# cwchenwang/outdoor-nerf-depth

Measured on AMD Instinct MI355X. Metric: train rays/sec, KITTI 375x1242, 64+128 samples/ray, higher is better.
Workload: dtype bf16 MFMA operands, f32 accumulate / f32 master weights

## Files before the change

### outdoor_nerf_depth_amd/csrc/nerfpp_common.h

```cpp
#pragma once
#include <stdint.h>
#ifdef NERFPP_PROBES
#include <stdlib.h>
#endif

namespace nerfpp {

constexpr int WIDTH = 256;
constexpr int FRAG_BYTES = 1024;
constexpr int BLK_FRAGS = 16;
constexpr int DIR_REF = 27;
constexpr int DIRW = 32;
constexpr int N_NET = 2;

__host__ __device__ constexpr int pe_dim(int net) { return net == 0 ? 3 : 4; }
__host__ __device__ constexpr int pe_ref_ch(int net) { return net == 0 ? 63 : 84; }
__host__ __device__ constexpr int kpe(int net) { return net == 0 ? 4 : 6; }
__host__ __device__ constexpr int kpew(int net) { return kpe(net) * 16; }

enum RefTensor { RT_L0 = 0, RT_SIGMA = 8, RT_REMAP = 9, RT_RGB0 = 10, RT_RGB1 = 11, RT_COUNT = 12 };
__host__ __device__ constexpr int ref_out(int t) {
  return t < 8 ? 256 : t == RT_SIGMA ? 1 : t == RT_REMAP ? 256 : t == RT_RGB0 ? 128 : 3;
}
__host__ __device__ constexpr int ref_in(int net, int t) {
  return t == 0 ? pe_ref_ch(net) : t == 5 ? pe_ref_ch(net) + 256 : t < 8 ? 256
       : t == RT_SIGMA ? 256 : t == RT_REMAP ? 256 : t == RT_RGB0 ? 256 + DIR_REF : 128;
}
__host__ __device__ constexpr int ref_w_off(int net, int t) {
  int off = 0;
  for (int i = 0; i < t; ++i) off += ref_out(i) * ref_in(net, i) + ref_out(i);
  return off;
}
__host__ __device__ constexpr int ref_b_off(int net, int t) {
  return ref_w_off(net, t) + ref_out(t) * ref_in(net, t);
}
__host__ __device__ constexpr int net_params(int net) { return ref_w_off(net, RT_COUNT); }
constexpr int FG_PARAMS = net_params(0);
constexpr int BG_PARAMS = net_params(1);
constexpr int LEVEL_PARAMS = FG_PARAMS + BG_PARAMS;
static_assert(FG_PARAMS == 595844 && BG_PARAMS == 606596, "reference parameter count");

enum FwdStage { FS_L0 = 0, FS_L5 = 5, FS_REMAP = 8, FS_SIG = 9, FS_RGB0 = 10, FS_RGB1 = 11, FS_COUNT = 12 };
__host__ __device__ constexpr int fs_nob(int s) { return s <= FS_REMAP ? 8 : s == FS_RGB0 ? 4 : 1; }
__host__ __device__ constexpr int fs_nkc(int net, int s) {
  return s == FS_L0 ? kpe(net) : s == FS_L5 ? kpe(net) + 16 : s == FS_REMAP ? 0 : s < FS_REMAP ? 16
       : s == FS_SIG ? 16 : s == FS_RGB0 ? 20 : 16;
}
constexpr int DERIVED_WC = 128 * 256;
constexpr int DERIVED_FLOATS = DERIVED_WC + 128;
__host__ __device__ constexpr int fs_frags(int net, int s) { return fs_nob(s) * fs_nkc(net, s); }
__host__ __device__ constexpr int fs_frag_off(int net, int s) {
  int off = 0;
  for (int i = 0; i < s; ++i) off += fs_frags(net, i);
  return off;
}
__host__ __device__ constexpr int fs_bias_off(int s) {
  int off = 0;
  for (int i = 0; i < s; ++i) off += fs_nob(i) * 32;
  return off;
}
__host__ __device__ constexpr int fwd_frags(int net) { return fs_frag_off(net, FS_COUNT); }
constexpr int FWD_BIAS_FLOATS = fs_bias_off(FS_COUNT);
static_assert(fwd_frags(0) % BLK_FRAGS == 0 && fwd_frags(1) % BLK_FRAGS == 0, "block aligned");

enum BwdStage { BS_DG = 0, BS_DR = 1, BS_DH7 = 2, BS_COUNT = 10 };
__host__ __device__ constexpr int bs_nob(int s) { return s == BS_DG ? 4 : 8; }
__host__ __device__ constexpr int bs_nkc(int s) { return s == BS_DG ? 4 : s == BS_DR ? 0 : s == BS_DH7 ? 10 : 16; }
__host__ __device__ constexpr int bs_frags(int s) { return bs_nob(s) * bs_nkc(s); }
__host__ __device__ constexpr int bs_frag_off(int s) {
  int off = 0;
  for (int i = 0; i < s; ++i) off += bs_frags(i);
  return off;
}
constexpr int BWD_FRAGS = bs_frag_off(BS_COUNT);
static_assert(BWD_FRAGS % BLK_FRAGS == 0, "block aligned");
__host__ __device__ constexpr int bs_layer(int s) { return 10 - s; }

__host__ __device__ constexpr int w_planes(int P) { return P == 1 ? 1 : 2; }
__host__ __device__ constexpr int a_planes(int P) { return P == 2 ? 2 : 1; }
__host__ __device__ constexpr size_t fwd_stream_bytes(int net, int P) { return (size_t)fwd_frags(net) * FRAG_BYTES * w_planes(P); }
__host__ __device__ constexpr size_t bwd_stream_bytes(int P) { return (size_t)BWD_FRAGS * FRAG_BYTES * w_planes(P); }

__host__ __device__ constexpr int kslot(int c, int hi, int t) { return 16 * c + 8 * (t >> 2) + 4 * hi + (t & 3); }
__host__ __device__ constexpr int dfeat(int ob, int hi, int r) { return ob * 32 + (r & 3) + 8 * (r >> 2) + 4 * hi; }

__host__ __device__ constexpr int pe_ref_of_lane_slot(int D, int hi, int m) {
  const int nf = 10 * D;
  if (m < nf) {
    const int k = 5 * hi + m / (2 * D), d = (m % (2 * D)) / 2, s = m & 1;
    return D + k * 2 * D + s * D + d;
  }
  const int id = 2 * hi + (m - nf);
  return (m - nf) < 2 && id < D ? id : -1;
}
__host__ __device__ constexpr int dir_ref_of_lane_slot(int hi, int m) {
  if (m < 12) {
    const int k = 2 * hi + m / 6, d = (m % 6) / 2, s = m & 1;
    return 3 + k * 6 + s * 3 + d;
  }
  const int id = 2 * hi + (m - 12);
  return (m - 12) < 2 && id < 3 ? id : -1;
}
__host__ __device__ constexpr int feat_hi(int f) { return ((f % 16) / 4) % 2; }
__host__ __device__ constexpr int feat_m(int f) { return 8 * (f / 16) + 4 * ((f % 16) / 8) + (f % 4); }
__host__ __device__ constexpr int pe_ref_of_feat(int net, int f) { return pe_ref_of_lane_slot(pe_dim(net), feat_hi(f), feat_m(f)); }
__host__ __device__ constexpr int dir_ref_of_feat(int f) { return dir_ref_of_lane_slot(feat_hi(f), feat_m(f)); }

enum Tensor {
  T_X = 0, T_H0 = 1,  T_R = 9, T_G = 10, T_DIRX = 11,
  T_DZ0 = 12,  T_DR = 20, T_DS = 21, T_DG = 22, T_DP = 23, T_COUNT = 24
};
constexpr int DSG_LD = 160, DG_COL0 = 32;
__host__ __device__ constexpr int tensor_ld(int net, int t) {
  return t == T_X ? kpew(net) : (t >= T_H0 && t <= T_R) ? 256 : t == T_G ? 128 : t == T_DIRX ? 32
       : (t >= T_DZ0 && t <= T_DR) ? 256 : (t == T_DS || t == T_DG) ? DSG_LD : 32;
}
__host__ __device__ constexpr int tensor_off_cols(int net, int t) {
  int off = 0;
  for (int i = 0; i < t; ++i) off += tensor_ld(net, i);
  return off;
}
__host__ __device__ constexpr int ws_cols(int net) { return tensor_off_cols(net, T_COUNT); }

__host__ __device__ constexpr int gw_O(int s) { return s <= FS_REMAP ? 256 : s == FS_SIG ? 32 : s == FS_RGB0 ? 128 : 32; }
__host__ __device__ constexpr int gw_I(int net, int s) {
  return s == FS_L0 ? kpew(net) : s == FS_L5 ? kpew(net) + 256 : s <= FS_SIG ? 256 : s == FS_RGB0 ? 256 + DIRW : 128;
}
__host__ __device__ constexpr int gw_off(int net, int s) {
  int off = 0;
  for (int i = 0; i < s; ++i) off += gw_O(i) * gw_I(net, i);
  return off;
}
__host__ __device__ constexpr int gw_floats(int net) { return gw_off(net, FS_COUNT); }
__host__ __device__ constexpr int gb_off(int s) {
  int off = 0;
  for (int i = 0; i < s; ++i) off += gw_O(i);
  return off;
}
constexpr int GB_FLOATS = gb_off(FS_COUNT);
__host__ __device__ constexpr int gslab_floats(int net) { return gw_floats(net) + GB_FLOATS; }
__host__ __device__ constexpr int gw_dz_tensor(int s) {
  return s < 8 ? T_DZ0 + s : s == FS_REMAP ? T_DR : s == FS_SIG ? T_DS : s == FS_RGB0 ? T_DG : T_DP;
}

struct DwJob {
  int16_t a_tensor, b_tensor;
  int16_t b_tensor2, n_i1;
  int16_t o0, i0;
  int16_t n_o, n_i;
  int32_t gw_off;
  int16_t gw_ld;
  int16_t gb_off;
  int16_t o_split;
  int16_t gw_ld2, gb_off2;
  int32_t gw_off2;
};
constexpr int DW_JOBS = 10;
constexpr int DW_KMAX = 64;

// ... 161 lines not shown
```

### outdoor_nerf_depth_amd/csrc/nerfpp_mlp.hip

```cpp
#include <hip/hip_runtime.h>
#include <math.h>
#include <stdint.h>
#include <type_traits>
#include <utility>
#include "hip_device.h"
#include "nerfpp_common.h"
#include "nerfpp_kernels.h"

#ifdef NERFPP_PROBES
#include "nerfpp_mlp_probes.h"
#else
namespace nerfpp { namespace probe {
constexpr int STAMP_BYTES = 0;
__device__ __forceinline__ void stamp(int, int, int, int, uint32_t) {}
__device__ __forceinline__ void dump_stamps(uint32_t, int, int) {}
}}
#endif

namespace nerfpp {

using hipdev::bf16x8, hipdev::bf16x2, hipdev::f16x8, hipdev::f16x2, hipdev::f32x2, hipdev::f32x4, hipdev::f32x8, hipdev::f32x16;
using hipdev::u32x4, hipdev::s16x2, hipdev::s16x8, hipdev::glds16xN_saddr;
#define LDS_AS __attribute__((address_space(3)))

template <int P> struct Frag { bf16x8 v[a_planes(P)]; };

extern __shared__ __attribute__((aligned(16))) char smem[];

enum { PIPE_RING = 1, PIPE_ROLES = 2 };

__device__ __forceinline__ uint32_t lds_base_addr() { return (uint32_t)(uintptr_t)(LDS_AS char*)smem; }

template <int P, int NW, int MODE, int NBUF, int BF = BLK_FRAGS>
struct WeightPipe {
  static constexpr int BLKF = BF;
  static constexpr int BLK_BYTES = BF * P * FRAG_BYTES;
  static constexpr int SHARE = MODE == PIPE_ROLES ? BF * P : BF * P / NW;
  static constexpr int AHEAD = NBUF - 1;
  static_assert(AHEAD >= 1 && AHEAD <= 3 && (AHEAD - 1) * SHARE < 63, "ring depth");
  const char* g;
  uint32_t stamp_off = 0;
  int nblk, cur, step, wave, lane;
  int slot_cur, slot_issue, next_issue;
  uint32_t lds_base;
  __device__ __forceinline__ void init(const void* stream, int nblk_, int wave_, int lane_) {
    g = (const char*)stream; nblk = nblk_; cur = 0; step = 0; wave = wave_; lane = lane_;
    slot_cur = 0; slot_issue = 0; next_issue = 0;
    lds_base = lds_base_addr();
#pragma unroll
    for (int b = 0; b < AHEAD; ++b) issue();
  }
  static constexpr bool TRICKLE = MODE == PIPE_RING && AHEAD >= 2;
  int pend_blk = -1, pend_slot = 0;
  __device__ __forceinline__ void issue_frags(int blk, int slot, int f0, int f1) {
    if (MODE == PIPE_ROLES && wave != 0) return;
    const int w0 = MODE == PIPE_ROLES ? 0 : wave * SHARE;
    const char* sb = g + (size_t)blk * BLK_BYTES + (size_t)w0 * FRAG_BYTES;
    const uint32_t dst = lds_base + slot * BLK_BYTES + w0 * FRAG_BYTES;
#pragma unroll
    for (int f = f0; f < f1; f += 4) {
      const int n = f1 - f < 4 ? f1 - f : 4;
      const char* a = sb + f * FRAG_BYTES;
      const uint32_t d = dst + f * FRAG_BYTES;
      if (n == 4) glds16xN_saddr<4>(a, (uint32_t)lane * 16u, d);
      else if (n == 3) glds16xN_saddr<3>(a, (uint32_t)lane * 16u, d);
      else if (n == 2) glds16xN_saddr<2>(a, (uint32_t)lane * 16u, d);
      else glds16xN_saddr<1>(a, (uint32_t)lane * 16u, d);
    }
  }
  __device__ __forceinline__ bool claim(int& blk, int& slot) {
    blk = next_issue; slot = slot_issue;
    ++next_issue;
    slot_issue = slot_issue + 1 == NBUF ? 0 : slot_issue + 1;
    return blk < nblk;
  }
  __device__ __forceinline__ void issue() {
    int blk, slot;
    if (!claim(blk, slot)) return;
    static_assert(SHARE == 2 || SHARE % 4 == 0, "per-wave fragment count");
    issue_frags(blk, slot, 0, SHARE);
  }
  __device__ __forceinline__ void trickle(int i, int n) {
    if constexpr (TRICKLE) {
      if (pend_blk < 0) return;
      issue_frags(pend_blk, pend_slot, SHARE * i / n, SHARE * (i + 1) / n);
    }
  }
  __device__ __forceinline__ void wait_counted() {
    const int younger = nblk - 1 - step < AHEAD - 1 ? nblk - 1 - step : AHEAD - 1;
    if (AHEAD >= 3 && younger >= 2) asm volatile("s_waitcnt vmcnt(%0)" ::"n"(2 * SHARE) : "memory");
    else if (AHEAD >= 2 && younger == 1) asm volatile("s_waitcnt vmcnt(%0)" ::"n"(SHARE) : "memory");
    else asm volatile("s_waitcnt vmcnt(0)" ::: "memory");
  }
  __device__ __forceinline__ void sync_step() {
    probe::stamp(0, cur, wave, lane, stamp_off);
    if constexpr (MODE == PIPE_RING) {
      wait_counted();
      __builtin_amdgcn_s_barrier();
    } else {
      if (wave == 0) wait_counted();
      asm volatile("s_waitcnt lgkmcnt(0)" ::: "memory");
      __builtin_amdgcn_s_barrier();
    }
    probe::stamp(1, cur, wave, lane, stamp_off);
    if constexpr (TRICKLE) { int b_, s_; pend_blk = claim(b_, s_) ? b_ : -1; pend_slot = s_; }
    else issue();
    ++step;
  }
  __device__ __forceinline__ const char* acquire() {
    sync_step();
    const char* l = smem + slot_cur * BLK_BYTES + lane * 16;
    slot_cur = slot_cur + 1 == NBUF ? 0 : slot_cur + 1;
    ++cur;
    return l;
  }
};

template <int P>
__device__ __forceinline__ void mfma_p(f32x16& acc, const char* lfrag, const Frag<P>& b) {
  const bf16x8 a_hi = *(const bf16x8*)(lfrag);
  if constexpr (P == 3) {
    const bf16x8 a_lo = *(const bf16x8*)(lfrag + FRAG_BYTES);
    const f16x8 bb = __builtin_bit_cast(f16x8, b.v[0]);
    acc = __builtin_amdgcn_mfma_f32_32x32x16_f16(__builtin_bit_cast(f16x8, a_hi), bb, acc, 0, 0, 0);
    acc = __builtin_amdgcn_mfma_f32_32x32x16_f16(__builtin_bit_cast(f16x8, a_lo), bb, acc, 0, 0, 0);
  } else {
    acc = __builtin_amdgcn_mfma_f32_32x32x16_bf16(a_hi, b.v[0], acc, 0, 0, 0);
  }
}

struct NoHook { __device__ __forceinline__ void operator()(int) const {} };
#define HOOK(...) [&](int blk) __attribute__((always_inline)) { __VA_ARGS__; }
#define IC(n) std::integral_constant<int, (n)>{}

constexpr int LDS_PREFETCH = 4;
constexpr int LDS_PREFETCH_SPLIT = 4;
constexpr int CHAIN_GROUP = 4;

template <int NOB, int NKC, int P, int LIVE = NKC, typename Pipe, typename Hook>
__device__ __forceinline__ void stage_gemm(Pipe& pipe, f32x16 (&acc)[NOB], const Frag<P> (&b)[NKC], const Hook& hook) {
  static_assert(P == 1 || P == 3, "split-bf16 runs stage_units (nerfpp_mlp_split.h)");
  constexpr int KPB = Pipe::BLKF / NOB;
  static_assert(NKC % KPB == 0, "stage must be block aligned");
  static_assert(LIVE >= 1 && LIVE <= NKC, "live k-chunks");
#pragma unroll
// ... 118 lines not shown
      }
      const s16x8 zero = {0, 0, 0, 0, 0, 0, 0, 0};
      h[2 * ob + hh].v[0] = __builtin_bit_cast(bf16x8, __builtin_elementwise_max(__builtin_bit_cast(s16x8, d), zero));
    }
  return make_uint4(m[0], m[1], m[2], m[3]);
}

template <int N, int P>
__device__ __forceinline__ void zero_invalid(Frag<P> (&f)[N], bool valid) {
#pragma unroll
  for (int c = 0; c < N; ++c)
#pragma unroll
    for (int p = 0; p < a_planes(P); ++p) {
      u32x4 d = __builtin_bit_cast(u32x4, f[c].v[p]);
#pragma unroll
      for (int w = 0; w < 4; ++w) d[w] = valid ? d[w] : 0u;
      f[c].v[p] = __builtin_bit_cast(bf16x8, d);
    }
}

template <int NOB>
__device__ __forceinline__ void init_bias_lds(f32x16 (&acc)[NOB], uint32_t lds_off_bytes, int hi) {
  LDS_AS char* base = (LDS_AS char*)smem;
#pragma unroll
  for (int ob = 0; ob < NOB; ++ob) {
#pragma unroll
    for (int q = 0; q < 4; ++q) {
      const f32x4 v = *(LDS_AS f32x4*)(base + lds_off_bytes + (ob * 32 + hi * 16 + 4 * q) * 4);
      acc[ob][4 * q] = v[0]; acc[ob][4 * q + 1] = v[1]; acc[ob][4 * q + 2] = v[2]; acc[ob][4 * q + 3] = v[3];
    }
  }
}
template <int NOB>
__device__ __forceinline__ void init_zero(f32x16 (&acc)[NOB]) {
#pragma unroll
  for (int ob = 0; ob < NOB; ++ob)
#pragma unroll
    for (int r = 0; r < 16; ++r) acc[ob][r] = 0.f;
}

__device__ __forceinline__ void store_nt16(char* gptr, const uint4 v) {
  const u32x4 vv = {v.x, v.y, v.z, v.w};
  __builtin_nontemporal_store(vv, (u32x4*)gptr);
}

constexpr int REGION_MASK = 16 * FRAG_BYTES;
constexpr int REGION_BYTES = REGION_MASK + 1024;

__device__ __forceinline__ char* frag_addr(__bf16* base, int ld, size_t wave_row0, int c, int lane) {
  const size_t blk = (wave_row0 >> 5) * (size_t)(ld >> 4) + (size_t)c;
  return (char*)base + blk * FRAG_BYTES + ((((lane & 31) << 1) | (lane >> 5)) << 4);
}
template <int P>
__device__ __forceinline__ void store_chunk(__bf16* base, size_t plane, int ld, size_t wave_row0, int lane, int c, const Frag<P>& f, int np = a_planes(P)) {
#pragma unroll
  for (int p = 0; p < a_planes(P); ++p)
    if (p < np) store_nt16(frag_addr(base + p * plane, ld, wave_row0, c, lane), saved_image<P>(*(const uint4*)&f.v[p]));
}
template <int NCH, int P>
__device__ __forceinline__ void save_frags(__bf16* base, size_t plane, int ld, size_t wave_row0, int lane, const Frag<P> (&h)[NCH], int np = a_planes(P)) {
  __builtin_amdgcn_sched_barrier(0);
#pragma unroll
  for (int c = 0; c < NCH; ++c) store_chunk<P>(base, plane, ld, wave_row0, lane, c, h[c], np);
  __builtin_amdgcn_sched_barrier(0);
}

template <int NCH, int P>
__device__ __forceinline__ void handoff_write(char* region, int lane, const Frag<P> (&h)[NCH]) {
  static_assert(a_planes(P) == 1, "one plane");
#pragma unroll
  for (int c = 0; c < NCH; ++c) *(uint4*)(region + (c * 64 + lane) * 16) = *(const uint4*)&h[c].v[0];
}
template <int P>
__device__ __forceinline__ void handoff_flush_one(const char* region, int lane, __bf16* base, int ld, size_t row0, int cr, int ct) {
  static_assert(a_planes(P) == 1, "one plane");
  store_nt16(frag_addr(base, ld, row0, ct, lane), saved_image<P>(*(const uint4*)(region + (cr * 64 + lane) * 16)));
}
template <int P>
__device__ __forceinline__ void handoff_flush_chunks(const char* region, int lane, __bf16* base, int ld, size_t row0, int c0, int n) {
#pragma unroll 4
  for (int c = c0; c < c0 + n; ++c) handoff_flush_one<P>(region, lane, base, ld, row0, c, c);
}

template <int NOB>
__device__ __forceinline__ void mask_to_frags(const f32x16 (&acc)[NOB], const uint4 bits, Frag<1> (&dz)[2 * NOB]) {
  const uint32_t act[4] = {~bits.x, ~bits.y, ~bits.z, ~bits.w};
#pragma unroll
  for (int ob = 0; ob < NOB; ++ob)
#pragma unroll
    for (int hh = 0; hh < 2; ++hh) {
      u32x4 d;
#pragma unroll
      for (int w = 0; w < 4; ++w) d[w] = pack2<1>(acc[ob][8 * hh + 2 * w], acc[ob][8 * hh + 2 * w + 1]);
#pragma unroll
      for (int w = 0; w < 4; ++w) {
        const int j = (ob & 1) * 8 + hh * 4 + w;
        const s16x2 keep = __builtin_bit_cast(s16x2, act[ob >> 1] << j) >> (s16x2){15, 15};
        d[w] &= __builtin_bit_cast(uint32_t, keep);
      }
      dz[2 * ob + hh].v[0] = __builtin_bit_cast(bf16x8, d);
    }
}

template <int NET>
__device__ __forceinline__ void sample_point(const MlpGeom& gm, size_t row, int S, float (&x)[4], float (&vd)[3],
                                             float* depth_real) {
#pragma clang fp contract(off)
  const int ray = (int)(row / S);
  const float ox = gm.ray_o[ray * 3], oy = gm.ray_o[ray * 3 + 1], oz = gm.ray_o[ray * 3 + 2];
  const float dx = gm.ray_d[ray * 3], dy = gm.ray_d[ray * 3 + 1], dz = gm.ray_d[ray * 3 + 2];
  const float z = gm.z[row];
  const float dd = dx * dx + dy * dy + dz * dz;
  const float inv_n = 1.f / sqrtf(dd);
  vd[0] = dx * inv_n; vd[1] = dy * inv_n; vd[2] = dz * inv_n;
  if (NET == 0) {
    x[0] = ox + z * dx; x[1] = oy + z * dy; x[2] = oz + z * dz; x[3] = 0.f;
    *depth_real = 0.f;
  } else {
    const float d1 = -(dx * ox + dy * oy + dz * oz) / dd;
    const float mx = ox + d1 * dx, my = oy + d1 * dy, mz = oz + d1 * dz;
    const float pmn = sqrtf(mx * mx + my * my + mz * mz);
    const float d2 = sqrtf(1.f - pmn * pmn) * inv_n;
    const float sx = ox + (d1 + d2) * dx, sy = oy + (d1 + d2) * dy, sz = oz + (d1 + d2) * dz;
    float ax = oy * sz - oz * sy, ay = oz * sx - ox * sz, az = ox * sy - oy * sx;
    const float an = 1.f / sqrtf(ax * ax + ay * ay + az * az);
    ax *= an; ay *= an; az *= an;
    const float phi = asinf(pmn), theta = asinf(pmn * z);
    float sn, cs;
    sincosf(phi - theta, &sn, &cs);
    const float cx = ay * sz - az * sy, cy = az * sx - ax * sz, cz = ax * sy - ay * sx;
    const float dt = (ax * sx + ay * sy + az * sz) * (1.f - cs);
    float nx = sx * cs + cx * sn + ax * dt, ny = sy * cs + cy * sn + ay * dt, nz = sz * cs + cz * sn + az * dt;
    const float nn = 1.f / sqrtf(nx * nx + ny * ny + nz * nz);
    x[0] = nx * nn; x[1] = ny * nn; x[2] = nz * nn; x[3] = z;
    *depth_real = 1.f / (z + 1e-6f) * cosf(theta) * inv_n + d1;
  }
}

template <int P>
__device__ __forceinline__ void pe_sincos(float arg, float* sn, float* cs) {
#pragma clang fp contract(off)
  if constexpr (P != 2) {
    const float r = __builtin_amdgcn_fractf(arg * 0.15915494309189535f);
    *sn = __builtin_amdgcn_sinf(r);
    *cs = __builtin_amdgcn_cosf(r);
  } else {
    const float n = __builtin_rintf(arg * 0.6366197723675814f);
    float r = __builtin_fmaf(-n, 1.5707962512969971f, arg);
    r = __builtin_fmaf(-n, 7.5497901264043321e-08f, r);
    r = __builtin_fmaf(-n, -1.7763568394002505e-15f, r);
    const float z = r * r;
    float ps = __builtin_fmaf(z, 2.7183114e-6f, -0.00019839335f);
    ps = __builtin_fmaf(z, ps, 0.008333329f);
    ps = __builtin_fmaf(z, ps, -0.16666667f);
    const float s = __builtin_fmaf(r * z, ps, r);
    float pc = __builtin_fmaf(z, 2.4390449e-5f, -0.0013886763f);
    pc = __builtin_fmaf(z, pc, 0.04166662f);
    pc = __builtin_fmaf(z, pc, -0.5f);
    const float c = __builtin_fmaf(z, pc, 1.0f);
    const int q = (int)n;
    const float ss = (q & 1) ? c : s, cc = (q & 1) ? s : c;
    *sn = (q & 2) ? -ss : ss;
    *cs = ((q + 1) & 2) ? -cc : cc;
  }
}

template <int NET, int P>
__device__ __forceinline__ void encode_point(const float (&x)[4], int hi, Frag<P> (&pe)[kpe(NET)]) {
#pragma clang fp contract(off)
  constexpr int D = pe_dim(NET), NV = kpe(NET) * 8;
  float v[NV];
#pragma unroll
  for (int kk = 0; kk < 5; ++kk) {
    const float scale = __int_as_float((127 + 5 * hi + kk) << 23);
#pragma unroll
    for (int d = 0; d < D; ++d) {
      float sn, cs;
      pe_sincos<P>(x[d] * scale, &sn, &cs);
      v[(kk * D + d) * 2] = sn;
      v[(kk * D + d) * 2 + 1] = cs;
    }
  }
  v[10 * D] = hi ? x[2] : x[0];
  v[10 * D + 1] = hi ? (D == 4 ? x[3] : 0.f) : x[1];
// ... 200 lines not shown
      for (int c = 0; c < KPE; ++c) in5[c] = pe2[c];
    }
#pragma unroll
    for (int c = 0; c < 16; ++c) in5[KPE + c] = h[c];
    bias_init8(acc, fs_bias_off(FS_L5));
    stage_gemm<8, KPE + 16, P>(pipe, acc, in5, HOOK(psave_h(blk, h, a.ws.t[T_H0 + 4], 4)));
    const uint4 bits = acc_to_frags_relu_bits<8, P>(acc, h);
    finish_h(h, bits, 5);
  }
  for (int l = 6; l <= 7; ++l) {
    bias_init8(acc, fs_bias_off(FS_L0) + l * 256);
    stage_gemm<8, 16, P>(pipe, acc, h, HOOK(psave_h(blk, h, a.ws.t[T_H0 + l - 1], l - 1)));
    const uint4 bits = acc_to_frags_relu_bits<8, P>(acc, h);
    finish_h(h, bits, l);
  }
  f32x16 acc1[1];
  bias_init1(acc1, fs_bias_off(FS_SIG));
  constexpr int SIG_BLKS = P == 1 ? 1 : 0;
  stage_gemm<1, 16, P>(pipe, acc1, h, HOOK(if constexpr (P == 1) psave_hc(blk, h, a.ws.t[T_H0 + 7], 7, IC(3))));
  const float sigma_raw = acc1[0][0];
  Frag<P> g[8];
  {
    Frag<P> in[20];
#pragma unroll
    for (int c = 0; c < 16; ++c) in[c] = h[c];
    Frag<P> df[2];
    encode_dir<P>(vd, hi, df);
    in[16] = df[0]; in[17] = df[1]; in[18] = zero_frag<P>(); in[19] = zero_frag<P>();
    f32x16 acc4[4];
    bias_init4(acc4, fs_bias_off(FS_RGB0));
    stage_gemm<4, 20, P, 18>(pipe, acc4, in, HOOK(psave_hc(blk + SIG_BLKS, h, a.ws.t[T_H0 + 7], 7, IC(P == 1 ? 3 : 2))));
    const uint4 bits = acc_to_frags_relu_bits<4, P>(acc4, g);
    save(std::integral_constant<int, 8>{}, a.ws.t[T_G], 128, g, true, bits, 8);
  }
  {
    Frag<P> in[16];
#pragma unroll
    for (int c = 0; c < 8; ++c) in[c] = g[c];
#pragma unroll
    for (int c = 8; c < 16; ++c) in[c] = zero_frag<P>();
    bias_init1(acc1, fs_bias_off(FS_RGB1));
    stage_gemm<1, 16, P, 8>(pipe, acc1, in, HOOK(flush(blk, IC(8), a.ws.t[T_G], 128, 8)));
  }
  if (valid && hi == 0) {
    float4 o;
    o.x = 1.f / (1.f + expf(-acc1[0][0]));
    o.y = 1.f / (1.f + expf(-acc1[0][1]));
    o.z = 1.f / (1.f + expf(-acc1[0][2]));
    o.w = sigma_raw;
    ((float4*)a.out_raw)[row] = o;
    if (NET == 1) a.depth_real[row] = depth_real;
  }
  probe::dump_stamps(LD::TOTAL, wave, lane);
}

template <int NET, int NW>
__device__ __forceinline__ void mlp_bwd_body(const MlpBwdArgs& a, const int bid) {
  constexpr int P = 1;
  using LD = BwdLds<NW>;
  const int lane = threadIdx.x & 63, wave = __builtin_amdgcn_readfirstlane(threadIdx.x >> 6);
  const int hi = lane >> 5;
  const size_t row_raw = (size_t)bid * (NW * 32) + wave * 32 + (lane & 31);
  const bool valid = row_raw < (size_t)a.rows;
  const size_t row = valid ? row_raw : (size_t)a.rows - 1;
  const size_t plane_rows = a.rows_padded;
  const size_t wrow0 = (size_t)bid * (NW * 32) + wave * 32;
  const bool loader = wave == 0, partner = wave == 1;
  char* region = smem + LD::REGION;
  const size_t tile_row0 = wrow0 - (size_t)wave * 32;
  const size_t nblk32 = a.rows_padded / 32;
  const uint32_t lds0 = lds_base_addr();

  auto issue_masks = [&](int mstage) __attribute__((always_inline)) {
    if (loader && mstage >= 0) {
      static_assert(NW % 4 == 0, "groups of four");
      const char* sb = (const char*)(a.masks + ((size_t)mstage * nblk32 + (size_t)bid * NW) * 64);
#pragma unroll
      for (int w = 0; w < NW; w += 4) glds16xN_saddr<4>(sb + w * 1024, (uint32_t)lane * 16u, lds0 + LD::MASKS + ((mstage & 1) * NW + w) * 1024);
    }
  };
  auto get_mask = [&](int mstage) __attribute__((always_inline)) -> uint4 {
    return *(const uint4*)(smem + LD::MASKS + ((mstage & 1) * NW + wave) * 1024 + lane * 16);
  };
  auto psave = [&](int blk, auto nch_c, const auto& frags, __bf16* base, int ld) __attribute__((always_inline)) {
    constexpr int NCH = decltype(nch_c)::value, HMAX = NW >= 5 ? 4 : NW - 1, HN = NCH / 4 < HMAX ? NCH / 4 : HMAX;
    constexpr int Q = (NCH + HN - 1) / HN, CPB = LD::BF / 8;
    if (a.skip_dz7 && base == a.ws.t[T_DZ0 + 7]) return;
    if (loader) {
      if (blk == 0) handoff_write<NCH, P>(region, lane, frags);
    } else {
      if (CPB * blk < NCH) {
#pragma unroll
        for (int i = 0; i < CPB; ++i)
          store_chunk<P>(base, plane_rows * ld, ld, wrow0, lane, CPB * blk + i, frags[CPB * blk + i]);
      }
      if (wave <= HN && blk == 2) handoff_flush_chunks<P>(region, lane, base, ld, tile_row0, Q * (wave - 1), Q);
    }
  };

  issue_masks(8);
  issue_masks(7);
  WeightPipe<P, NW, PIPE_ROLES, LD::NBUF, LD::BF> pipe;
  pipe.stamp_off = LD::TOTAL;
  pipe.init(a.w_stream, BWD_FRAGS / LD::BF, wave, lane);

  float4 d = ((const float4*)a.d_out)[row];
  if (!valid) d = make_float4(0.f, 0.f, 0.f, 0.f);
  auto save_dp_ds = [&](const float4& dd, size_t r0) __attribute__((always_inline)) {
    Frag<P> t[2];
    t[0] = zero_frag<P>(); t[1] = zero_frag<P>();
    if (hi == 0) { set_slot<P>(t[0], 0, dd.x); set_slot<P>(t[0], 1, dd.y); set_slot<P>(t[0], 2, dd.z); }
    save_frags<2, P>(a.ws.t[T_DP], plane_rows * 32, 32, r0, lane, t);
    t[0] = zero_frag<P>();
    if (hi == 0) set_slot<P>(t[0], 0, dd.w);
    save_frags<2, P>(a.ws.t[T_DS], plane_rows * DSG_LD, DSG_LD, r0, lane, t);
  };
  {
    const size_t rr = row_raw - 32;
    const bool ok = partner && rr < (size_t)a.rows;
    float4 d0 = make_float4(0.f, 0.f, 0.f, 0.f);
    if (ok) d0 = ((const float4*)a.d_out)[rr];
    if (!loader) save_dp_ds(d, wrow0);
    if (partner) save_dp_ds(d0, wrow0 - 32);
  }

  Frag<P> dg[8];
  {
    Frag<P> in[4];
#pragma unroll
    for (int c = 0; c < 4; ++c) in[c] = zero_frag<P>();
    if (hi == 0) { set_slot<P>(in[0], 0, d.x); set_slot<P>(in[0], 1, d.y); set_slot<P>(in[0], 2, d.z); }
    f32x16 acc4[4];
    init_zero<4>(acc4);
    stage_gemm<4, 4, P, 1>(pipe, acc4, in, NoHook{});
    mask_to_frags<4>(acc4, get_mask(8), dg);
  }
  f32x16 acc[8];
  Frag<P> dz[16];
  {
    Frag<P> in[10];
#pragma unroll
    for (int c = 0; c < 8; ++c) in[c] = dg[c];
    in[8] = zero_frag<P>(); in[9] = zero_frag<P>();
    if (hi == 0) set_slot<P>(in[8], 0, d.w);
    init_zero<8>(acc);
    stage_gemm<8, 10, P, 9>(pipe, acc, in, HOOK(psave(blk, IC(8), dg, a.ws.t[T_DG], DSG_LD); if (blk == 0) issue_masks(6)));
    mask_to_frags<8>(acc, get_mask(7), dz);
  }
  for (int l = 7; l >= 1; --l) {
    init_zero<8>(acc);
    stage_gemm<8, 16, P>(pipe, acc, dz, HOOK(psave(blk, IC(16), dz, a.ws.t[T_DZ0 + l], 256); if (blk == 0) issue_masks(l - 2)));
    mask_to_frags<8>(acc, get_mask(l - 1), dz);
  }
  save_frags<16, P>(a.ws.t[T_DZ0], plane_rows * 256, 256, wrow0, lane, dz);
  probe::dump_stamps(LD::TOTAL, wave, lane);
}

}
#include "nerfpp_mlp_split.h"
namespace nerfpp {

template <int P, int NW, bool TRAIN>
__global__ __launch_bounds__(NW * 64, (NW == 8 ? 2 : 1)) void mlp_fwd_pair_kernel(MlpFwdArgs a0, MlpFwdArgs a1, int tiles0) {
  if constexpr (P == 2) {
    const bool fg = (int)blockIdx.x < tiles0;
    const bool hi_only = TRAIN && !(fg ? a0.save_lo : a1.save_lo);
    if (fg) { if (hi_only) mlp_fwd_body_split<0, NW, TRAIN, TRAIN>(a0, (int)blockIdx.x); else mlp_fwd_body_split<0, NW, TRAIN, false>(a0, (int)blockIdx.x); }
    else { if (hi_only) mlp_fwd_body_split<1, NW, TRAIN, TRAIN>(a1, (int)blockIdx.x - tiles0); else mlp_fwd_body_split<1, NW, TRAIN, false>(a1, (int)blockIdx.x - tiles0); }
  } else {
    if ((int)blockIdx.x < tiles0) mlp_fwd_body<0, P, NW, TRAIN>(a0, (int)blockIdx.x);
    else mlp_fwd_body<1, P, NW, TRAIN>(a1, (int)blockIdx.x - tiles0);
  }
}
template <int P, int NW>
__global__ __launch_bounds__(NW * 64, (P == 1 ? 2 : 1)) void mlp_bwd_pair_kernel(MlpBwdArgs a0, MlpBwdArgs a1, int tiles0) {
  if constexpr (P == 2) {
    if ((int)blockIdx.x < tiles0) mlp_bwd_body_split<0, NW>(a0, (int)blockIdx.x);
    else mlp_bwd_body_split<1, NW>(a1, (int)blockIdx.x - tiles0);
  } else {
    if ((int)blockIdx.x < tiles0) mlp_bwd_body<0, NW>(a0, (int)blockIdx.x);
    else mlp_bwd_body<1, NW>(a1, (int)blockIdx.x - tiles0);
  }
}

}

using namespace nerfpp;

constexpr int WAVES_P1 = 8;
#define MLP_WAVES(P) ((P) == 1 ? WAVES_P1 : (P) == 3 ? 8 : 4)

template <int P, bool TRAIN>
static void launch_fwd_t(hipStream_t st, const MlpFwdArgs& a0, const MlpFwdArgs& a1, int which) {
  constexpr int NW = MLP_WAVES(P);
  const int tile = NW * 32;
  const int t0 = which == 2 ? 0 : (int)((a0.rows + tile - 1) / tile), t1 = which == 1 ? 0 : (int)((a1.rows + tile - 1) / tile);
  constexpr size_t l0 = FwdLds<0, P, NW, TRAIN>::TOTAL, l1 = FwdLds<1, P, NW, TRAIN>::TOTAL;
  constexpr size_t lds = (l0 > l1 ? l0 : l1) + probe::STAMP_BYTES;
  static_assert(lds <= 160 * 1024, "LDS budget");
  hipLaunchKernelGGL((mlp_fwd_pair_kernel<P, NW, TRAIN>), dim3(t0 + t1), dim3(NW * 64), lds, st, a0, a1, t0);
}
template <int P>
static void launch_bwd_t(hipStream_t st, const MlpBwdArgs& a0, const MlpBwdArgs& a1, int which) {
  constexpr int NW = MLP_WAVES(P);
  const int tile = NW * 32;
  const int t0 = which == 2 ? 0 : (int)((a0.rows + tile - 1) / tile), t1 = which == 1 ? 0 : (int)((a1.rows + tile - 1) / tile);
  constexpr size_t lds = (P == 2 ? (size_t)BwdLdsV2<NW>::TOTAL : (size_t)BwdLds<NW>::TOTAL) + probe::STAMP_BYTES;
  static_assert(lds <= 160 * 1024, "LDS budget");
  hipLaunchKernelGGL((mlp_bwd_pair_kernel<P, NW>), dim3(t0 + t1), dim3(NW * 64), lds, st, a0, a1, t0);
}

#ifndef NERFPP_MLP_PART
#define NERFPP_MLP_PART -1
#endif
#define MLP_PART(k) (NERFPP_MLP_PART == -1 || NERFPP_MLP_PART == (k))
#define FWD_ENTRY(P, TRAIN) void launch_fwd_##P##_##TRAIN(hipStream_t st, const MlpFwdArgs& a0, const MlpFwdArgs& a1, int which)
#define BWD_ENTRY(P) void launch_bwd_##P(hipStream_t st, const MlpBwdArgs& a0, const MlpBwdArgs& a1, int which)
FWD_ENTRY(1, 0); FWD_ENTRY(2, 0); FWD_ENTRY(1, 1); FWD_ENTRY(2, 1); FWD_ENTRY(3, 0); FWD_ENTRY(3, 1);
BWD_ENTRY(1); BWD_ENTRY(2);
#if MLP_PART(0)
FWD_ENTRY(1, 0) { launch_fwd_t<1, false>(st, a0, a1, which); }
#endif
#if MLP_PART(1)
FWD_ENTRY(2, 0) { launch_fwd_t<2, false>(st, a0, a1, which); }
#endif
#if MLP_PART(2)
FWD_ENTRY(1, 1) { launch_fwd_t<1, true>(st, a0, a1, which); }
#endif
#if MLP_PART(3)
FWD_ENTRY(2, 1) { launch_fwd_t<2, true>(st, a0, a1, which); }
#endif
#if MLP_PART(4)
BWD_ENTRY(1) { launch_bwd_t<1>(st, a0, a1, which); }
#endif
#if MLP_PART(5)
BWD_ENTRY(2) { launch_bwd_t<2>(st, a0, a1, which); }
// ... 20 lines not shown
```

Measured before the change: 489,100.

## Overlap backward dX-chain masking with next layer's GEMM via half-stage block reordering

Reorders the backward weight stream for the 256->256 layers so each 16-fragment block covers four output blocks across four k-chunks. That lets the second half of a layer's outputs be masked and converted while the first half of the next layer's GEMM runs. The ReLU-mask/bf16 conversion is split per output block and interleaved with the MFMAs using sched_group_barrier, and the handoff save is shifted to later blocks. This targets the serial conversion bubble between stages, at the cost of scattered global reads for the weight stream, extra register pressure and a non-unrolled layer loop.

```diff
diff --git a/outdoor_nerf_depth_amd/csrc/nerfpp_common.h b/outdoor_nerf_depth_amd/csrc/nerfpp_common.h
--- a/outdoor_nerf_depth_amd/csrc/nerfpp_common.h
+++ b/outdoor_nerf_depth_amd/csrc/nerfpp_common.h
@@ -75,6 +75,47 @@
 constexpr int BWD_FRAGS = bs_frag_off(BS_COUNT);
 static_assert(BWD_FRAGS % BLK_FRAGS == 0, "block aligned");
 __host__ __device__ constexpr int bs_layer(int s) { return 10 - s; }
+
+__host__ __device__ constexpr int hs_blocks(int nkc) { return nkc * 8 / BLK_FRAGS; }
+__host__ __device__ constexpr int hs_ob0(int nkc, int b) { return 4 * (b / (nkc / 4)); }
+__host__ __device__ constexpr int hs_kc(int nkc, int b, int g) { return 4 * (b % (nkc / 4)) + g; }
+__host__ __device__ constexpr int hs_group_frag(int nkc, int b, int g) { return hs_kc(nkc, b, g) * 8 + hs_ob0(nkc, b); }
+__host__ __device__ constexpr bool hs_map_ok(int nkc) {
+  if (nkc % 4 != 0 || nkc > 32) return false;
+  int seen[32 * 8] = {};
+  int last_kc[8] = {-1, -1, -1, -1, -1, -1, -1, -1};
+  for (int b = 0; b < hs_blocks(nkc); ++b)
+    for (int g = 0; g < 4; ++g)
+      for (int o = 0; o < 4; ++o) {
+        const int f = hs_group_frag(nkc, b, g) + o, kc = f / 8, ob = f % 8;
+        if (f < 0 || f >= nkc * 8 || kc != hs_kc(nkc, b, g) || ob != hs_ob0(nkc, b) + o) return false;
+        if (seen[f]++ != 0 || kc <= last_kc[ob]) return false;
+        last_kc[ob] = kc;
+      }
+  for (int f = 0; f < nkc * 8; ++f)
+    if (seen[f] != 1) return false;
+  return true;
+}
+static_assert(hs_map_ok(16), "half-stage block map of a 256 -> 256 stage");
+constexpr int BWD_HS_BLK0 = bs_frag_off(3) / BLK_FRAGS;
+static_assert(bs_frag_off(3) % BLK_FRAGS == 0 && bs_frags(3) == 16 * 8 && BWD_FRAGS == bs_frag_off(3) + 7 * 16 * 8, "B3..B9");
+struct BwdHalfStageMap {
+  __host__ __device__ static constexpr int group_frag(int blk, int g) {
+    return blk < BWD_HS_BLK0 ? blk * BLK_FRAGS + 4 * g
+         : bs_frag_off(3) + (blk - BWD_HS_BLK0) / 8 * 128 + hs_group_frag(16, (blk - BWD_HS_BLK0) % 8, g);
+  }
+};
+__host__ __device__ constexpr bool bwd_hs_stream_ok() {
+  int seen[BWD_FRAGS] = {};
+  for (int blk = 0; blk < BWD_FRAGS / BLK_FRAGS; ++blk)
+    for (int g = 0; g < 4; ++g)
+      for (int o = 0; o < 4; ++o) {
+        const int f = BwdHalfStageMap::group_frag(blk, g) + o;
+        if (f < 0 || f >= BWD_FRAGS || seen[f]++ != 0) return false;
+      }
+  return true;
+}
+static_assert(bwd_hs_stream_ok(), "every fragment of the dX chain's stream is fetched exactly once");
 
 __host__ __device__ constexpr int w_planes(int P) { return P == 1 ? 1 : 2; }
 __host__ __device__ constexpr int a_planes(int P) { return P == 2 ? 2 : 1; }
diff --git a/outdoor_nerf_depth_amd/csrc/nerfpp_mlp.hip b/outdoor_nerf_depth_amd/csrc/nerfpp_mlp.hip
--- a/outdoor_nerf_depth_amd/csrc/nerfpp_mlp.hip
+++ b/outdoor_nerf_depth_amd/csrc/nerfpp_mlp.hip
@@ -31,9 +31,11 @@
 
 __device__ __forceinline__ uint32_t lds_base_addr() { return (uint32_t)(uintptr_t)(LDS_AS char*)smem; }
 
-template <int P, int NW, int MODE, int NBUF, int BF = BLK_FRAGS>
+template <int P, int NW, int MODE, int NBUF, int BF = BLK_FRAGS, typename MAP = void>
 struct WeightPipe {
   static constexpr int BLKF = BF;
+  static constexpr bool MAPPED = !std::is_void<MAP>::value;
+  static_assert(!MAPPED || (MODE == PIPE_ROLES && P == 1 && BF % 4 == 0), "block maps: the loader of the bf16 roles pipe");
   static constexpr int BLK_BYTES = BF * P * FRAG_BYTES;
   static constexpr int SHARE = MODE == PIPE_ROLES ? BF * P : BF * P / NW;
   static constexpr int AHEAD = NBUF - 1;
@@ -61,6 +63,7 @@
     for (int f = f0; f < f1; f += 4) {
       const int n = f1 - f < 4 ? f1 - f : 4;
       const char* a = sb + f * FRAG_BYTES;
+      if constexpr (MAPPED) a = g + (size_t)MAP::group_frag(blk, f / 4) * FRAG_BYTES;
       const uint32_t d = dst + f * FRAG_BYTES;
       if (n == 4) glds16xN_saddr<4>(a, (uint32_t)lane * 16u, d);
       else if (n == 3) glds16xN_saddr<3>(a, (uint32_t)lane * 16u, d);
@@ -345,24 +348,80 @@
   for (int c = c0; c < c0 + n; ++c) handoff_flush_one<P>(region, lane, base, ld, row0, c, c);
 }
 
+__device__ __forceinline__ void mask_ob_to_frags(const f32x16& acc, const uint32_t act, const int ob, Frag<1>& c0, Frag<1>& c1) {
+#pragma unroll
+  for (int hh = 0; hh < 2; ++hh) {
+    u32x4 d;
+#pragma unroll
+    for (int w = 0; w < 4; ++w) d[w] = pack2<1>(acc[8 * hh + 2 * w], acc[8 * hh + 2 * w + 1]);
+#pragma unroll
+    for (int w = 0; w < 4; ++w) {
+      const int j = (ob & 1) * 8 + hh * 4 + w;
+      const s16x2 keep = __builtin_bit_cast(s16x2, act << j) >> (s16x2){15, 15};
+      d[w] &= __builtin_bit_cast(uint32_t, keep);
+    }
+    (hh ? c1 : c0).v[0] = __builtin_bit_cast(bf16x8, d);
+  }
+}
 template <int NOB>
 __device__ __forceinline__ void mask_to_frags(const f32x16 (&acc)[NOB], const uint4 bits, Frag<1> (&dz)[2 * NOB]) {
   const uint32_t act[4] = {~bits.x, ~bits.y, ~bits.z, ~bits.w};
 #pragma unroll
-  for (int ob = 0; ob < NOB; ++ob)
-#pragma unroll
-    for (int hh = 0; hh < 2; ++hh) {
-      u32x4 d;
-#pragma unroll
-      for (int w = 0; w < 4; ++w) d[w] = pack2<1>(acc[ob][8 * hh + 2 * w], acc[ob][8 * hh + 2 * w + 1]);
-#pragma unroll
-      for (int w = 0; w < 4; ++w) {
-        const int j = (ob & 1) * 8 + hh * 4 + w;
-        const s16x2 keep = __builtin_bit_cast(s16x2, act[ob >> 1] << j) >> (s16x2){15, 15};
-        d[w] &= __builtin_bit_cast(uint32_t, keep);
+  for (int ob = 0; ob < NOB; ++ob) mask_ob_to_frags(acc[ob], act[ob >> 1], ob, dz[2 * ob], dz[2 * ob + 1]);
+}
+
+constexpr int HS_VALU_PER_OB = 32;
+__device__ __forceinline__ void pin_frag(Frag<1>& f) {
+  u32x4 d = __builtin_bit_cast(u32x4, f.v[0]);
+  asm volatile("" : "+v"(d));
+  f.v[0] = __builtin_bit_cast(bf16x8, d);
+}
+template <typename Pipe, typename GetBits, typename Hook>
+__device__ __forceinline__ void half_stage_gemm_bwd(Pipe& pipe, f32x16 (&acc)[8], Frag<1> (&b)[16], Frag<1> (&nxt)[8],
+                                                    const uint4 prev_bits, uint4& bits, const GetBits& get_bits, const Hook& hook) {
+  static_assert(Pipe::BLKF == 16 && Pipe::MAPPED, "16-fragment blocks through the half-stage block map");
+  const uint32_t pact[2] = {~prev_bits.z, ~prev_bits.w};
+  auto block = [&](auto blk_c) __attribute__((always_inline)) {
+    constexpr int blk = decltype(blk_c)::value, ob0 = hs_ob0(16, blk);
+    constexpr int NCONV = blk >= 4 ? 1 : blk < 2 ? 2 : 0;
+    const char* l = pipe.acquire();
+    if constexpr (blk == 0 || blk == 4) {
+#pragma unroll
+      for (int o = 0; o < 4; ++o)
+#pragma unroll
+        for (int r = 0; r < 16; ++r) acc[ob0 + o][r] = 0.f;
+    }
+    if constexpr (blk < 2) {
+#pragma unroll
+      for (int i = 0; i < 2; ++i) {
+        constexpr int ob = 4 + 2 * blk;
+        mask_ob_to_frags(acc[ob + i], pact[(ob + i - 4) >> 1], ob + i, b[2 * (ob + i)], b[2 * (ob + i) + 1]);
       }
-      dz[2 * ob + hh].v[0] = __builtin_bit_cast(bf16x8, d);
-    }
+    }
+    if constexpr (blk == 3) bits = get_bits();
+    if constexpr (blk >= 4) {
+      constexpr int ob = blk - 4;
+      mask_ob_to_frags(acc[ob], ob < 2 ? ~bits.x : ~bits.y, ob, nxt[2 * ob], nxt[2 * ob + 1]);
+    }
+#pragma unroll
+    for (int kl = 0; kl < 4; ++kl)
+#pragma unroll
+      for (int o = 0; o < 4; ++o) mfma_p<1>(acc[ob0 + o], l + (kl * 4 + o) * FRAG_BYTES, b[hs_kc(16, blk, kl)]);
+    constexpr int D = LDS_PREFETCH, VPM = (NCONV * HS_VALU_PER_OB + 15) / 16;
+    if constexpr (blk == 3) __builtin_amdgcn_sched_group_barrier(0x100, 1, 0);
+#pragma unroll
+    for (int i = 0; i < D; ++i) __builtin_amdgcn_sched_group_barrier(0x100, 1, 0);
+#pragma unroll
+    for (int i = 0; i < 16; ++i) {
+      __builtin_amdgcn_sched_group_barrier(0x008, 1, 0);
+      if constexpr (VPM > 0) __builtin_amdgcn_sched_group_barrier(0x002, VPM, 0);
+      if (i < 16 - D) __builtin_amdgcn_sched_group_barrier(0x100, 1, 0);
+    }
+    if constexpr (blk < 2) { pin_frag(b[16 + 4 * blk - 8]); pin_frag(b[17 + 4 * blk - 8]); pin_frag(b[18 + 4 * blk - 8]); pin_frag(b[19 + 4 * blk - 8]); }
+    if constexpr (blk >= 4) { pin_frag(nxt[2 * (blk - 4)]); pin_frag(nxt[2 * (blk - 4) + 1]); }
+    hook(blk);
+  };
+  block(IC(0)); block(IC(1)); block(IC(2)); block(IC(3)); block(IC(4)); block(IC(5)); block(IC(6)); block(IC(7));
 }
 
 template <int NET>
@@ -729,25 +788,25 @@
   auto get_mask = [&](int mstage) __attribute__((always_inline)) -> uint4 {
     return *(const uint4*)(smem + LD::MASKS + ((mstage & 1) * NW + wave) * 1024 + lane * 16);
   };
-  auto psave = [&](int blk, auto nch_c, const auto& frags, __bf16* base, int ld) __attribute__((always_inline)) {
+  auto psave = [&](int blk, auto nch_c, const auto& frags, __bf16* base, int ld, int hblk = 0) __attribute__((always_inline)) {
     constexpr int NCH = decltype(nch_c)::value, HMAX = NW >= 5 ? 4 : NW - 1, HN = NCH / 4 < HMAX ? NCH / 4 : HMAX;
     constexpr int Q = (NCH + HN - 1) / HN, CPB = LD::BF / 8;
     if (a.skip_dz7 && base == a.ws.t[T_DZ0 + 7]) return;
     if (loader) {
-      if (blk == 0) handoff_write<NCH, P>(region, lane, frags);
+      if (blk == hblk) handoff_write<NCH, P>(region, lane, frags);
     } else {
       if (CPB * blk < NCH) {
 #pragma unroll
         for (int i = 0; i < CPB; ++i)
           store_chunk<P>(base, plane_rows * ld, ld, wrow0, lane, CPB * blk + i, frags[CPB * blk + i]);
       }
-      if (wave <= HN && blk == 2) handoff_flush_chunks<P>(region, lane, base, ld, tile_row0, Q * (wave - 1), Q);
+      if (wave <= HN && blk == hblk + 2) handoff_flush_chunks<P>(region, lane, base, ld, tile_row0, Q * (wave - 1), Q);
     }
   };
 
   issue_masks(8);
   issue_masks(7);
-  WeightPipe<P, NW, PIPE_ROLES, LD::NBUF, LD::BF> pipe;
+  WeightPipe<P, NW, PIPE_ROLES, LD::NBUF, LD::BF, BwdHalfStageMap> pipe;
   pipe.stamp_off = LD::TOTAL;
   pipe.init(a.w_stream, BWD_FRAGS / LD::BF, wave, lane);
 
@@ -792,13 +851,22 @@
     if (hi == 0) set_slot<P>(in[8], 0, d.w);
     init_zero<8>(acc);
     stage_gemm<8, 10, P, 9>(pipe, acc, in, HOOK(psave(blk, IC(8), dg, a.ws.t[T_DG], DSG_LD); if (blk == 0) issue_masks(6)));
-    mask_to_frags<8>(acc, get_mask(7), dz);
-  }
+  }
+  uint4 prev_bits = get_mask(7);
+#pragma unroll
+  for (int ob = 0; ob < 4; ++ob) mask_ob_to_frags(acc[ob], ob < 2 ? ~prev_bits.x : ~prev_bits.y, ob, dz[2 * ob], dz[2 * ob + 1]);
+#pragma nounroll
   for (int l = 7; l >= 1; --l) {
-    init_zero<8>(acc);
-    stage_gemm<8, 16, P>(pipe, acc, dz, HOOK(psave(blk, IC(16), dz, a.ws.t[T_DZ0 + l], 256); if (blk == 0) issue_masks(l - 2)));
-    mask_to_frags<8>(acc, get_mask(l - 1), dz);
-  }
+    uint4 bits;
+    Frag<P> nxt[8];
+    half_stage_gemm_bwd(pipe, acc, dz, nxt, prev_bits, bits, [&]() __attribute__((always_inline)) { return get_mask(l - 1); },
+                        HOOK(psave(blk, IC(16), dz, a.ws.t[T_DZ0 + l], 256, 2); if (blk == 0) issue_masks(l - 2)));
+#pragma unroll
+    for (int c = 0; c < 8; ++c) dz[c] = nxt[c];
+    prev_bits = bits;
+  }
+#pragma unroll
+  for (int ob = 4; ob < 8; ++ob) mask_ob_to_frags(acc[ob], ob < 6 ? ~prev_bits.z : ~prev_bits.w, ob, dz[2 * ob], dz[2 * ob + 1]);
   save_frags<16, P>(a.ws.t[T_DZ0], plane_rows * 256, 256, wrow0, lane, dz);
   probe::dump_stamps(LD::TOTAL, wave, lane);
 }
```

Result: no change. 493,500 (median of 5 runs) (+0.9%).
